# ddemidov/amgcl

Hardware: NVIDIA H100
Metric: cg_iterations_per_second (higher is better)
Workload: dtype f64

## Files before the change

### amgcl_b200/csrc/api_matrices.cu

```cuda
#include "internal.cuh"
#include "csr_kernels.cuh"
#include "csr_launch.cuh"
#include "window.cuh"
#include "offsets.cuh"
#include "patterns.cuh"
#include "narrow.cuh"
#include "values.cuh"

namespace b200 {
int tail_enqueue_csr(b200_ctx_t ctx, int mode, b200_csr_t A, const CsrArgsT<PrecDD> &a);
bool small_csr_accepts(b200_ctx_t ctx, b200_csr_t A);
int small_csr_launch(b200_ctx_t ctx, int mode, b200_csr_t A, const CsrArgsT<PrecDD> &a);
}

using namespace b200;

namespace b200 {

static int choose_lanes(double avg) {
    if (avg <= 12.0) return 1;
    if (avg <= 40.0) return 2;
    if (avg <= 64.0) return 4;
    if (avg <= 160.0) return 8;
    if (avg <= 320.0) return 16;
// ... 427 lines not shown
    A->rows_dist = rd; A->cols_dist = cd;
    A->gather_rows = !rd;
    A->row_off = rows.lo(rank); A->row_B = rows.B;
    A->n_loc = sp.n_loc;
#define DCSR_CUDA(call)                                                        \
    do {                                                                       \
        cudaError_t rc__ = (call);                                             \
        if (rc__ != cudaSuccess) {                                             \
            csr_free(A);                                                       \
            return cuda_fail(rc__, #call, __FILE__, __LINE__);                 \
        }                                                                      \
    } while (0)
    if (cd) {
        A->S = sp.S;
        A->n_send = (int64_t)sp.send_idx.size();
        std::vector<int32_t> idx(sp.send_idx.begin(), sp.send_idx.end());
        DCSR_CUDA(cudaMalloc(&A->send_idx, std::max<size_t>(1, idx.size()) * sizeof(int)));
        const size_t halo_n = std::max<size_t>(2, (size_t)(P * sp.S));
        DCSR_CUDA(cudaMalloc(&A->halo_owned, halo_n * sizeof(double)));
        A->halo = A->halo_owned;
        DCSR_CUDA(cudaMemsetAsync(A->halo, 0, halo_n * sizeof(double), ctx->stream));
        if (!idx.empty())
            DCSR_CUDA(cudaMemcpyAsync(A->send_idx, idx.data(), idx.size() * sizeof(int),
                                      cudaMemcpyHostToDevice, ctx->stream));
        A->bytes += idx.size() * sizeof(int) + (size_t)(P * sp.S) * sizeof(double);
        for (int q = 0; q < P; ++q)
            A->xchg[q] = q != rank && (sp.dep[(size_t)rank * P + q] || sp.dep[(size_t)q * P + rank]);
    }
    if (A->gather_rows && !ctx->p2p) {
        DCSR_CUDA(cudaMalloc((void **)&A->ybuf, ((size_t)P * (size_t)rows.B + 2) * sizeof(double)));
        DCSR_CUDA(cudaMemsetAsync(A->ybuf, 0, ((size_t)P * (size_t)rows.B + 2) * sizeof(double), ctx->stream));
        A->bytes += (size_t)P * (size_t)rows.B * sizeof(double);
    }
    DCSR_CUDA(cudaStreamSynchronize(ctx->stream));
#undef DCSR_CUDA
    if (ctx->p2p) {
        if (cd) {
            size_t half = (size_t)P * (size_t)A->S * sizeof(double);
            half = (std::max<size_t>(half, 16) + 255) & ~size_t(255);
            A->pb_half = half;
            rc = peer_alloc(ctx, kFlagBytes + 2 * half, &A->pb_local, A->pb_peer);
            if (rc) {
                csr_free(A);
                return rc;
            }
            A->bytes += kFlagBytes + 2 * half;
        }
        if (A->gather_rows) {
            size_t half = (size_t)P * (size_t)rows.B * sizeof(double);
            half = (std::max<size_t>(half, 16) + 255) & ~size_t(255);
            A->gb_half = half;
            rc = peer_alloc(ctx, kFlagBytes + 2 * half, &A->gb_local, A->gb_peer);
            if (rc) {
                csr_free(A);
                return rc;
            }
            A->bytes += kFlagBytes + 2 * half;
        }
    }
    *out = A;
    return B200_OK;
}

template <int MODE, int L, bool HALO, class P>
static int launch_csr_LH(b200_ctx_t ctx, b200_csr_t A, const CsrArgsT<P> &args) {
    constexpr bool fp64 = std::is_same<P, PrecDD>::value;
    const StageLayout lay = stage_layout(A->rows_cap, A->nnz_cap, (int)sizeof(typename P::TV));
    if (fp64 && ctx->opt_spmv_variant == 0 && !HALO) {
        const int smem = kHeaderBytes + lay.bytes;
        static bool attr_set[64] = {};
        if (!attr_set[ctx->device & 63]) {
            B200_CUDA(cudaFuncSetAttribute(csr_block_kernel<MODE, L, HALO, PrecDD>,
                                           cudaFuncAttributeMaxDynamicSharedMemorySize, 200 * 1024));
            attr_set[ctx->device & 63] = true;
        }
        csr_block_kernel<MODE, L, HALO, PrecDD><<<(unsigned)A->nblocks, kThreads, smem, ctx->stream>>>(
            *reinterpret_cast<const CsrArgsT<PrecDD> *>(&args));
    } else {
        int rc = B200_OK;
        bool done = false;
        const int fmt = launch_format<P>(ctx, A);
        if constexpr (L <= 4 && !HALO && !IndexedValues<typename P::TV>::value) {
            if (fmt == FMT_PATVAL) {
                rc = launch_ring_pv<MODE, L, P>(ctx, A, args);
                done = true;
            }
        }
        if constexpr (L <= 4) {
            if (fmt == FMT_PATTERN) {
                rc = launch_ring_pat<MODE, L, HALO, P>(ctx, A, args);
                done = true;
            }
        }
        if constexpr (L <= 4) {
            if (fmt == FMT_OFFSET) {
                rc = launch_ring_off<MODE, L, HALO, P>(ctx, A, args);
                done = true;
            }
        }
        if constexpr (L <= 8 && !IndexedValues<typename P::TV>::value) {
            if (fmt == FMT_WINDOW) {
                rc = launch_ring_win<MODE, L, HALO, P>(ctx, A, args);
                done = true;
            }
        }
        if constexpr (L <= 8) {
            if (fmt == FMT_COL16) {
                rc = launch_ring_c16<MODE, L, HALO, P>(ctx, A, args);
                done = true;
            }
            if (fmt == FMT_COL24) {
                rc = launch_ring_c24<MODE, L, HALO, P>(ctx, A, args);
                done = true;
            }
        }
        if (!done) rc = launch_ring_impl<MODE, L, HALO, P, FMT_PLAIN>(ctx, A, args);
        if (rc) return rc;
    }
    B200_CHECK_LAUNCH();
    ctx->launches++;
    return B200_OK;
}

template <int MODE, int L, class P>
static int launch_csr_L(b200_ctx_t ctx, b200_csr_t A, const CsrArgsT<P> &args) {
    if constexpr (!IndexedValues<typename P::TV>::value) {
        if (args.xh) return launch_csr_LH<MODE, L, true, P>(ctx, A, args);
    }
    return launch_csr_LH<MODE, L, false, P>(ctx, A, args);
}

template <int MODE, class P>
static int launch_csr_lanes(b200_ctx_t ctx, b200_csr_t A, const CsrArgsT<P> &args) {
    if (ctx->recording) A->in_graph = true;
    ProfScope prof(ctx, MODE, A->nrows, A->ncols, A->nnz, launch_format<P>(ctx, A), (int)sizeof(typename P::TV));
    switch (A->lanes) {
    case 1:  return launch_csr_L<MODE, 1>(ctx, A, args);
    case 2:  return launch_csr_L<MODE, 2>(ctx, A, args);
    case 4:  return launch_csr_L<MODE, 4>(ctx, A, args);
    case 8:  return launch_csr_L<MODE, 8>(ctx, A, args);
    case 16: return launch_csr_L<MODE, 16>(ctx, A, args);
    default: return launch_csr_L<MODE, 32>(ctx, A, args);
    }
}

template <class PI>
static CsrArgsT<PI> indexed_args(b200_csr_t A, const CsrArgsT<PrecDD> &args) {
    CsrArgsT<PI> s;
    static_assert(sizeof(s) == sizeof(args), "indexed arguments differ from PrecDD only in the value type");
    memcpy(&s, &args, sizeof(s));
    s.val = static_cast<const typename PI::TV *>(A->vidx);
    s.vtab = A->vtab;
    s.vtab_n = A->vtab_n;
    return s;
}

template <int MODE, class P>
static int launch_csr(b200_ctx_t ctx, b200_csr_t A, const CsrArgsT<P> &args) {
    if (A->nblocks == 0) return B200_OK;
    if (std::is_same<P, PrecDD>::value && !args.ndot && !args.xh && !args.gather_on &&
        tail_accepts_csr(ctx, A))
        return tail_enqueue_csr(ctx, MODE, A, *reinterpret_cast<const CsrArgsT<PrecDD> *>(&args));
    {
        const int trc = tail_flush(ctx);
        if (trc) return trc;
    }
    if (std::is_same<P, PrecDD>::value && MODE != MODE_RESID_SCALED && !args.ndot && !args.xh &&
// ... 747 lines not shown
```

### amgcl_b200/csrc/api_patvals.cu

```cuda
#include "csr_launch.cuh"

namespace b200 {

template <int MODE, int L, class P>
int launch_ring_pv(b200_ctx_t ctx, b200_csr_t A, const CsrArgsT<P> &args) {
    return launch_ring_impl<MODE, L, false, P, FMT_PATVAL>(ctx, A, args);
}

#define B200_PV_INST(MODE, P)                                                                        \
    template int launch_ring_pv<MODE, 1, P>(b200_ctx_t, b200_csr_t, const CsrArgsT<P> &);            \
    template int launch_ring_pv<MODE, 2, P>(b200_ctx_t, b200_csr_t, const CsrArgsT<P> &);            \
    template int launch_ring_pv<MODE, 4, P>(b200_ctx_t, b200_csr_t, const CsrArgsT<P> &);

B200_PV_INST(MODE_SPMV, PrecDD)
B200_PV_INST(MODE_SPMV, PrecFF)
B200_PV_INST(MODE_SPMV, PrecFD)
B200_PV_INST(MODE_SPMV, PrecFFD)
B200_PV_INST(MODE_SPMV_ACC, PrecDD)
B200_PV_INST(MODE_SPMV_ACC, PrecFF)
B200_PV_INST(MODE_SPMV_ACC, PrecFD)
B200_PV_INST(MODE_SPMV_ACC, PrecFFD)
B200_PV_INST(MODE_RESID, PrecDD)
B200_PV_INST(MODE_RESID, PrecFF)
B200_PV_INST(MODE_RESID, PrecFD)
B200_PV_INST(MODE_RESID, PrecFDF)
B200_PV_INST(MODE_RESID_SCALED, PrecDD)
B200_PV_INST(MODE_RELAX, PrecDD)
B200_PV_INST(MODE_RELAX, PrecFF)
B200_PV_INST(MODE_RELAX, PrecFD)
B200_PV_INST(MODE_SPMV, PrecSD)
B200_PV_INST(MODE_SPMV_ACC, PrecSD)
B200_PV_INST(MODE_RESID, PrecSD)
B200_PV_INST(MODE_RESID_SCALED, PrecSD)
B200_PV_INST(MODE_RELAX, PrecSD)

}
```

### amgcl_b200/csrc/csr_kernels.cuh

```cuda
#pragma once
#include "common.cuh"
#include "reduce.cuh"
#include <type_traits>

namespace b200 {

enum { FMT_PLAIN = 0,
       FMT_WINDOW = 1,
       FMT_OFFSET = 2,
       FMT_PATTERN = 3,
       FMT_COL16 = 4,
       FMT_COL24 = 5,
       FMT_PATVAL = 6 };
static_assert(FMT_PLAIN == B200_FMT_PLAIN && FMT_WINDOW == B200_FMT_WINDOW && FMT_OFFSET == B200_FMT_OFFSET &&
              FMT_PATTERN == B200_FMT_PATTERN && FMT_COL16 == B200_FMT_COL16 && FMT_COL24 == B200_FMT_COL24 &&
              FMT_PATVAL == B200_FMT_PATVAL,
              "formats as include/amgcl_b200_formats.h reports them");

enum { MODE_SPMV = 0, MODE_SPMV_ACC = 1, MODE_RESID = 2, MODE_RELAX = 3,
       MODE_RESID_SCALED = 4 };

#ifndef B200_GATHER_BATCH
#define B200_GATHER_BATCH 4
#endif
// ... 11 lines not shown
typedef Prec<float, float, float, float, float>      PrecFF;
typedef Prec<float, double, double, double, float>   PrecFD;
typedef Prec<float, double, double, float, float>    PrecFDF;
typedef Prec<float, float, float, double, float>     PrecFFD;
typedef Prec<float, double, double, double, double>  PrecSD;
typedef Prec<unsigned char, double, double, double, double>  PrecI8D;
typedef Prec<unsigned short, double, double, double, double> PrecI16D;

template <class TV> struct IndexedValues : std::false_type {};
template <> struct IndexedValues<unsigned char> : std::true_type {};
template <> struct IndexedValues<unsigned short> : std::true_type {};

template <class TS, class TV>
__device__ __forceinline__ TS value_of(TV v, const double *vtab) {
    if constexpr (IndexedValues<TV>::value) return (TS)vtab[v];
    else return (TS)v;
}

template <class P>
struct CsrArgsT {
    const int    *ptr;
    const unsigned short *ptr16;
    const int    *col;
    const typename P::TV *val;
    const double *vtab;
    int           vtab_n;
    const int4   *blk;
    int           nrows;
    int           nblocks;
    int           rows_cap;
    int           nnz_cap;
    int           row_stream;
    const typename P::TX *x;
    const typename P::TX *xh;
    int           nloc;
    const unsigned long long *wait_flags;
    unsigned int              wait_mask;
    unsigned long long        wait_seq;
    const int                *send_idx;
    int                       n_send;
    int                       nranks;
    typename P::TX           *push_data[kMaxRanks];
    unsigned long long       *push_flag[kMaxRanks];
    unsigned int             *push_ticket;
    unsigned long long        push_seq;
    int                       gather_on;
    typename P::TY           *gather_data[kMaxRanks];
    unsigned long long       *gather_flag[kMaxRanks];
    unsigned int             *gather_ticket;
    unsigned long long        gather_seq;
    const unsigned short *col16;
    const int2   *wrun;
    const int2   *wblk;
    int           run_cap;
    const unsigned char *idx8;
    const int    *off_tab;
    const unsigned char  *pid;
    const unsigned short *pat_start;
    const int    *pat_off;
    int           pat_total;
    const typename P::TV *pat_val;
    const unsigned short *clo16;
    const unsigned char  *chi8;
    const int    *cbase;
    typename P::TY       *y;
    typename P::TX       *xw;
    const typename P::TF *f;
    const typename P::TD *d;
    double        alpha;
    double        beta;
    int           ndot;
    const double *w;
    RedOut        red;
};
typedef CsrArgsT<PrecDD> CsrArgs;

struct StageLayout {
    int val_off, col_off, hi_off, ptr_off, run_off, pid_off, bytes;
};
__host__ __device__ inline StageLayout stage_layout(int rows_cap, int nnz_cap, int val_size,
                                                    int fmt = FMT_PLAIN, int run_cap = 0) {
    StageLayout s;
    s.val_off = 0;
    const bool patval = fmt == FMT_PATVAL;
    int val_bytes = patval ? 0 : nnz_cap * val_size + 16;
    val_bytes = (val_bytes + 15) & ~15;
    s.col_off = s.val_off + val_bytes;
    const bool narrow = fmt == FMT_COL16 || fmt == FMT_COL24;
    int col_bytes = fmt == FMT_WINDOW || narrow ? (nnz_cap + 16) * 2
                  : fmt == FMT_OFFSET  ? (nnz_cap + 32)
                  : fmt == FMT_PATTERN || patval ? 0
                                       : (nnz_cap + 8) * 4;
    col_bytes = (col_bytes + 15) & ~15;
    s.hi_off = s.col_off + col_bytes;
    int hi_bytes = fmt == FMT_COL24 ? nnz_cap + 32 : 0;
    hi_bytes = (hi_bytes + 15) & ~15;
    s.ptr_off = s.hi_off + hi_bytes;
    int ptr_bytes = patval ? 0 : (rows_cap + 16) * 2;
    ptr_bytes = (ptr_bytes + 15) & ~15;
    s.run_off = s.ptr_off + ptr_bytes;
    int run_bytes = fmt == FMT_WINDOW ? (run_cap + 2) * 8 : 0;
    run_bytes = (run_bytes + 15) & ~15;
    s.pid_off = s.run_off + run_bytes;
    int pid_bytes = fmt == FMT_PATTERN || patval ? rows_cap + 32 : 0;
    pid_bytes = (pid_bytes + 15) & ~15;
    s.bytes = s.pid_off + pid_bytes;
    return s;
}
constexpr int kMaxStages   = 8;
constexpr int kHeaderBytes = 448;
constexpr int kWinRunLen   = 64;
constexpr int kOffTabLen   = 256;
constexpr int kPatCap      = 256;
constexpr int kPatOffCap   = 1024;
constexpr int kPatTabBytes = kPatOffCap * 4 + ((kPatCap + 1) * 2 + 15) / 16 * 16;
__host__ __device__ constexpr int fmt_table_bytes(int fmt, int val_size) {
    return fmt == FMT_OFFSET ? kOffTabLen * 4 : fmt == FMT_PATTERN ? kPatTabBytes
         : fmt == FMT_PATVAL ? kPatTabBytes + kPatOffCap * val_size : 0;
}

struct BlockDesc {
    int r0, r1;
    int e0, e1;
    int halo;
    int q0, q1;
    int cb;
};
static_assert(sizeof(BlockDesc) * kMaxStages <= 384 - 128, "descriptors overflow the header");

template <int FMT = FMT_PLAIN, class P>
__device__ __forceinline__ BlockDesc load_desc(const CsrArgsT<P> &a, int b) {
    const int4 q = __ldg(a.blk + b);
    BlockDesc d;
    d.halo = q.x < 0;
    d.r0 = q.x < 0 ? ~q.x : q.x;
    d.r1 = q.y; d.e0 = q.z; d.e1 = q.w;
    d.q0 = d.q1 = 0; d.cb = 0;
    if (FMT == FMT_WINDOW) {
        const int2 w = __ldg(a.wblk + b);
        d.q0 = w.x; d.q1 = w.y;
    }
    if (FMT == FMT_COL16 || FMT == FMT_COL24) d.cb = __ldg(a.cbase + b);
    return d;
}

template <int FMT = FMT_PLAIN, class P>
__device__ __forceinline__ bool issue_block(const CsrArgsT<P> &a, const BlockDesc &d, char *stage,
                                            const StageLayout &lay, uint64_t *bar,
                                            uint64_t policy) {
    typedef typename P::TV TV;
    constexpr int VA = 16 / (int)sizeof(TV);
    const int nnz = d.e1 - d.e0;
    if (FMT == FMT_PLAIN && nnz > a.nnz_cap) {
        asm volatile("mbarrier.arrive.shared::cta.b64 _, [%0];" ::"r"(ptx::smem_addr(bar))
                     : "memory");
        return false;
    }
    constexpr bool PV = FMT == FMT_PATVAL;
    const int a0 = d.e0 & ~(VA - 1);
    const int nval = PV ? 0 : ((d.e1 - a0) + VA - 1) & ~(VA - 1);
    const int p0 = d.r0 & ~7;
    const int nptr = PV ? 0 : ((d.r1 + 1 - p0) + 7) & ~7;
    int ncol = 0, nhi = 0, nrun = 0, npid = 0;
    const void *csrc = nullptr, *hsrc = nullptr, *psrc = nullptr;
    if (FMT == FMT_PLAIN) {
        const int c0 = d.e0 & ~3;
        ncol = (((d.e1 - c0) + 3) & ~3) * 4;
        csrc = a.col + c0;
    } else if (FMT == FMT_WINDOW || FMT == FMT_COL16 || FMT == FMT_COL24) {
        const int c0 = d.e0 & ~7;
        ncol = (((d.e1 - c0) + 7) & ~7) * 2;
        csrc = (FMT == FMT_WINDOW ? a.col16 : a.clo16) + c0;
    } else if (FMT == FMT_OFFSET) {
        const int c0 = d.e0 & ~15;
        ncol = ((d.e1 - c0) + 15) & ~15;
        csrc = a.idx8 + c0;
    }
    if (FMT == FMT_COL24) {
        const int h0 = d.e0 & ~15;
        nhi = ((d.e1 - h0) + 15) & ~15;
        hsrc = a.chi8 + h0;
    }
    if (FMT == FMT_WINDOW) {
        const int qa = d.q0 & ~1;
        nrun = (((d.q1 - qa) + 1) & ~1) * 8;
        psrc = a.wrun + qa;
    }
    if (FMT == FMT_PATTERN || PV) {
        const int q0 = d.r0 & ~15;
        npid = ((d.r1 - q0) + 15) & ~15;
        psrc = a.pid + q0;
    }
    const uint32_t bytes = nval * (int)sizeof(TV) + ncol + nhi + nptr * 2 + nrun + npid;
    ptx::mbar_expect_tx(bar, bytes);
    if (nval) ptx::bulk_g2s(stage + lay.val_off, a.val + a0, nval * (int)sizeof(TV), bar, policy);
    if (ncol) ptx::bulk_g2s(stage + lay.col_off, csrc, ncol, bar, policy);
    if (nhi) ptx::bulk_g2s(stage + lay.hi_off, hsrc, nhi, bar, policy);
    if (nptr) ptx::bulk_g2s(stage + lay.ptr_off, a.ptr16 + p0, nptr * 2, bar, policy);
    if (nrun) ptx::bulk_g2s(stage + lay.run_off, psrc, nrun, bar, policy);
    if (npid) ptx::bulk_g2s(stage + lay.pid_off, psrc, npid, bar, policy);
    return true;
}

struct RowAcc { double s0, s1; };

template <class P>
struct RowOps {
    typename P::TF f;
    typename P::TD d;
    typename P::TX x;
    typename P::TY y;
    double         w;
};
template <int MODE, class P>
__device__ __forceinline__ RowOps<P> load_row_ops(const CsrArgsT<P> &a, int r) {
    RowOps<P> o;
    o.f = 0; o.d = 0; o.x = 0; o.y = 0; o.w = 0.0;
    if (MODE == MODE_SPMV_ACC) o.y = a.y[r];
    if (MODE == MODE_RESID || MODE == MODE_RESID_SCALED || MODE == MODE_RELAX) o.f = a.f[r];
    if (MODE == MODE_RESID_SCALED || MODE == MODE_RELAX) o.d = a.d[r];
    if (MODE == MODE_RELAX) o.x = a.x[r];
    if (a.ndot && a.w) o.w = a.w[r];
    return o;
}

template <int MODE, class P>
__device__ __forceinline__ void store_row(const CsrArgsT<P> &a, int r, typename P::TY sum, RowAcc &acc,
                                          const RowOps<P> &o) {
    typedef typename P::TY TY;
    TY out;
    double wv = 0.0;
    if (MODE == MODE_SPMV) {
        out = (TY)(a.alpha * sum);
    } else if (MODE == MODE_SPMV_ACC) {
        out = (TY)(a.alpha * sum + a.beta * o.y);
    } else if (MODE == MODE_RESID) {
        out = (TY)(o.f - sum);
    } else if (MODE == MODE_RESID_SCALED) {
        const typename P::TF fr = o.f;
        out = (TY)(fr - sum);
        a.xw[r] = fma((typename P::TX)(a.alpha * o.d), (typename P::TX)fr, (typename P::TX)0);
    } else {
        const typename P::TF fr = o.f;
        const TY t = (TY)(fr - sum);
        const TY w = (TY)(a.alpha * o.d);
        out = fma(w, t, (TY)o.x);
        wv = (double)fr;
    }
    a.y[r] = out;
    if (a.gather_on) {
#pragma unroll 1
        for (int q = 0; q < a.nranks; ++q)
            if (a.gather_data[q]) a.gather_data[q][r] = out;
    }
    if (a.ndot) {
        const double yv = (double)out;
        if (a.w) wv = o.w;
        else if (MODE != MODE_RELAX) wv = yv;
        acc.s0 = fma(yv, wv, acc.s0);
        if (a.ndot > 1) acc.s1 = fma(yv, yv, acc.s1);
    }
}
template <int MODE, class P>
__device__ __forceinline__ void store_row(const CsrArgsT<P> &a, int r, typename P::TY sum, RowAcc &acc) {
    store_row<MODE>(a, r, sum, acc, load_row_ops<MODE>(a, r));
}

template <bool HALO, class P>
__device__ __forceinline__ typename P::TX gather(const CsrArgsT<P> &a,
                                                 const typename P::TX *__restrict__ x, int c) {
    if (HALO) {
        if (c < a.nloc) return __ldg(x + c);
        return __ldcg(a.xh + (c - a.nloc));
    }
    return __ldg(x + c);
}

template <int MODE, bool HALO, class P>
__device__ __forceinline__ typename P::TX gather_m(const CsrArgsT<P> &a,
                                                   const typename P::TX *__restrict__ x, int c) {
    typedef typename P::TX TX;
    if (MODE == MODE_RESID_SCALED)
        return fma((TX)(a.alpha * __ldg(a.d + c)), (TX)__ldg(a.f + c), (TX)0);
    return gather<HALO>(a, x, c);
}

template <bool HALO, class P>
__device__ __forceinline__ void wait_for_halo(const CsrArgsT<P> &a, const BlockDesc &d) {
    if (!HALO) return;
    if (!d.halo || !a.wait_mask) return;
    if (threadIdx.x == 0) {
        unsigned int m = a.wait_mask;
        while (m) {
            const int q = __ffs(m) - 1;
            m &= m - 1;
            unsigned long long v;
            do {
                asm volatile("ld.acquire.sys.global.u64 %0, [%1];" : "=l"(v) : "l"(a.wait_flags + q) : "memory");
            } while (v < a.wait_seq);
        }
    }
    __syncthreads();
}

template <int MODE, bool HALO, class P>
__device__ __forceinline__ void fill_window(const CsrArgsT<P> &a, const BlockDesc &d, const char *stage,
                                            const StageLayout &lay, typename P::TX *win) {
    const int2 *runs = reinterpret_cast<const int2 *>(stage + lay.run_off) + (d.q0 & 1);
    const int nq   = d.q1 - d.q0;
    const int lane = threadIdx.x & 31;
    const typename P::TX *__restrict__ x = a.x;
    for (int q = threadIdx.x >> 5; q < nq; q += kThreads / 32) {
        const int2 rn   = runs[q];
        const int first = rn.x;
        const int len   = rn.y & 0xffff;
        const int slot  = (int)((unsigned)rn.y >> 16);
#pragma unroll
        for (int i = lane; i < kWinRunLen; i += 32)
            if (i < len) win[slot + i] = gather_m<MODE, HALO>(a, x, first + i);
    }
    __syncthreads();
}

template <int MODE, int L, bool HALO, class P, int FMT = FMT_PLAIN>
__device__ __forceinline__ void compute_staged(const CsrArgsT<P> &a, const BlockDesc &d,
                                               const char *stage, const StageLayout &lay, RowAcc &acc,
                                               const typename P::TX *win = nullptr, const int *off = nullptr,
                                               const unsigned short *pstart = nullptr, int k0 = 0,
                                               const double *vtab = nullptr,
                                               const typename P::TV *pval = nullptr) {
    constexpr bool WIN = FMT == FMT_WINDOW;
    constexpr bool OFF = FMT == FMT_OFFSET;
    constexpr bool PV  = FMT == FMT_PATVAL;
    constexpr bool PAT = FMT == FMT_PATTERN || PV;
    constexpr bool NAR = FMT == FMT_COL16 || FMT == FMT_COL24;
    typedef typename P::TV TV;
    typedef typename P::TX TX;
    typedef typename P::TY TS;
    typedef typename std::conditional<WIN || NAR, unsigned short,
                                      typename std::conditional<OFF, unsigned char, int>::type>::type CI;
    static_assert(!((WIN || OFF || PAT || NAR) && L >= 16), "compressed column formats use at most 8 lanes per row");
    const unsigned char *pid_s = reinterpret_cast<const unsigned char *>(stage + lay.pid_off) + (d.r0 & 15);
    constexpr int VA = 16 / (int)sizeof(TV);
    const TV *val_s = reinterpret_cast<const TV *>(stage + lay.val_off);
    const CI     *col_s = reinterpret_cast<const CI *>(stage + lay.col_off);
    const unsigned char  *hi_s  = reinterpret_cast<const unsigned char *>(stage + lay.hi_off);
    const unsigned short *ptr_s = reinterpret_cast<const unsigned short *>(stage + lay.ptr_off) + (d.r0 & 7);
    const int vo = d.e0 & ~(VA - 1);
    const int nr = d.r1 - d.r0;
    const int co = WIN || NAR ? (d.e0 & ~7) : OFF ? (d.e0 & ~15) : (d.e0 & ~3);
    const int ho = d.e0 & ~15;
    auto stored_col = [&](int e) -> int {
        if (!NAR) return col_s[e - co];
        if (FMT == FMT_COL24) return d.cb + ((int)col_s[e - co] | (int)hi_s[e - ho] << 16);
        return d.cb + (int)col_s[e - co];
    };
    auto row_beg = [&](int rr) -> int { return d.e0 + (int)ptr_s[rr]; };
    auto row_end = [&](int rr) -> int { return d.e0 + (int)ptr_s[rr + 1] + (rr + 1 == nr ? d.e1 - d.e0 : 0); };
    constexpr int G = kThreads / L;
    const int c0   = (((int)threadIdx.x >> 5) - k0) & (kThreads / 32 - 1);
    const int g    = (threadIdx.x & 31) / L;
    const int lane = threadIdx.x % L;
    const TX *__restrict__ x = a.x;

    if (L >= 16) {
        constexpr int RU = kGatherBatch;
        for (int base = c0 * (32 / L); base < nr; base += G * RU) {
            int  beg[RU], end[RU], c[RU];
            TV   v[RU];
            TX   xv[RU];
            TS   sum[RU];
            bool rowok[RU], p[RU];
#pragma unroll
            for (int u = 0; u < RU; ++u) {
                const int rr = base + u * G + g;
                rowok[u] = rr < nr;
                beg[u] = rowok[u] ? row_beg(rr) : 0;
                end[u] = rowok[u] ? row_end(rr) : 0;
                sum[u] = 0;
            }
#pragma unroll
            for (int u = 0; u < RU; ++u) {
                const int e = beg[u] + lane;
                p[u] = e < end[u];
                c[u] = p[u] ? stored_col(e) : 0;
                v[u] = p[u] ? val_s[e - vo] : (TV)0;
            }
#pragma unroll
            for (int u = 0; u < RU; ++u) xv[u] = p[u] ? gather_m<MODE, HALO>(a, x, c[u]) : (TX)0;
#pragma unroll
            for (int u = 0; u < RU; ++u)
                if (p[u]) sum[u] = value_of<TS>(v[u], vtab) * (TS)xv[u];
#pragma unroll
            for (int u = 0; u < RU; ++u)
                for (int e = beg[u] + lane + L; e < end[u]; e += L)
                    sum[u] = fma(value_of<TS>(val_s[e - vo], vtab), (TS)gather_m<MODE, HALO>(a, x, stored_col(e)),
                                 sum[u]);
#pragma unroll
            for (int o = L / 2; o > 0; o >>= 1) {
#pragma unroll
                for (int u = 0; u < RU; ++u) sum[u] += __shfl_xor_sync(0xffffffffu, sum[u], o);
            }
#pragma unroll
            for (int u = 0; u < RU; ++u)
                if (rowok[u] && lane == 0) store_row<MODE>(a, d.r0 + base + u * G + g, sum[u], acc);
        }
    } else
    for (int base = c0 * (32 / L); base < nr; base += G) {
        const int  rr    = base + g;
        const bool valid = rr < nr;
        TS sum = 0;
        RowOps<P> ops;
        ops.f = 0; ops.d = 0; ops.x = 0; ops.y = 0; ops.w = 0.0;
        if (valid) {
            if (lane == 0) ops = load_row_ops<MODE>(a, d.r0 + rr);
            const int beg = PV ? (int)pstart[pid_s[rr]] : row_beg(rr);
            const int end = PV ? (int)pstart[pid_s[rr] + 1] : row_end(rr);
            int pb = 0;
            if (PAT && !PV) pb = (int)pstart[pid_s[rr]] - beg;
            constexpr int U = (L == 1) ? 2 * kGatherBatch : kGatherBatch;
            for (int e = beg + lane; e < end; e += U * L) {
                int  c[U];
                TX   xv[U];
                bool p[U];
#pragma unroll
                for (int u = 0; u < U; ++u) {
                    const int eu = e + u * L;
                    p[u] = eu < end;
                    if (PAT) c[u] = d.r0 + rr + off[pb + (p[u] ? eu : e)];
                    else c[u] = stored_col(p[u] ? eu : e);
                }
                if (OFF) {
#pragma unroll
                    for (int u = 0; u < U; ++u) c[u] = d.r0 + rr + off[c[u]];
                }
#pragma unroll
                for (int u = 0; u < U; ++u)
                    xv[u] = !p[u] ? (TX)0 : WIN ? win[c[u]] : gather_m<MODE, HALO>(a, x, c[u]);
#pragma unroll
                for (int u = 0; u < U; ++u)
                    if (p[u]) sum = fma(value_of<TS>(PV ? pval[e + u * L] : val_s[e + u * L - vo], vtab), (TS)xv[u], sum);
            }
        }
        if (L > 1) {
#pragma unroll
            for (int o = L / 2; o > 0; o >>= 1) sum += __shfl_xor_sync(0xffffffffu, sum, o);
        }
        if (valid && lane == 0) store_row<MODE>(a, d.r0 + rr, sum, acc, ops);
    }
}

template <int MODE, bool HALO, class P>
__device__ __forceinline__ void compute_long(const CsrArgsT<P> &a, const BlockDesc &d,
                                             double *red_s , RowAcc &acc) {
    typedef typename P::TX TX;
    typedef typename P::TY TS;
    const TX *__restrict__ x = a.x;
    for (int r = d.r0; r < d.r1; ++r) {
        const int beg = __ldg(a.ptr + r), end = __ldg(a.ptr + r + 1);
        TS sum = 0;
        for (int e = beg + threadIdx.x; e < end; e += kThreads)
            sum = fma(value_of<TS>(__ldg(a.val + e), a.vtab), (TS)gather_m<MODE, HALO>(a, x, __ldg(a.col + e)), sum);
#pragma unroll
        for (int o = 16; o > 0; o >>= 1) sum += __shfl_xor_sync(0xffffffffu, sum, o);
        __syncthreads();
        if ((threadIdx.x & 31) == 0) red_s[threadIdx.x >> 5] = (double)sum;
        __syncthreads();
        if (threadIdx.x == 0) {
            TS tot = 0;
#pragma unroll
            for (int w = 0; w < kThreads / 32; ++w) tot += (TS)red_s[w];
            store_row<MODE>(a, r, tot, acc);
        }
    }
}

__device__ __forceinline__ void xchg_st_release_sys(unsigned long long *p, unsigned long long v) {
    asm volatile("st.release.sys.global.u64 [%0], %1;" ::"l"(p), "l"(v) : "memory");
}
template <class P>
__device__ __forceinline__ void halo_push(const CsrArgsT<P> &a) {
    if (!a.push_seq) return;
    const typename P::TX *__restrict__ x = a.x;
    for (int i = blockIdx.x * kThreads + threadIdx.x; i < a.n_send; i += gridDim.x * kThreads) {
        const typename P::TX v = x[a.send_idx[i]];
#pragma unroll 1
        for (int q = 0; q < a.nranks; ++q)
            if (a.push_data[q]) a.push_data[q][i] = v;
    }
    __threadfence_system();
    __shared__ bool push_last;
    __syncthreads();
    if (threadIdx.x == 0) {
        const unsigned int done = atomicAdd(a.push_ticket, 1u);
        push_last = (done == gridDim.x - 1);
    }
    __syncthreads();
    if (push_last) {
        if (threadIdx.x < a.nranks && a.push_flag[threadIdx.x])
            xchg_st_release_sys(a.push_flag[threadIdx.x], a.push_seq);
        if (threadIdx.x == 0) *a.push_ticket = 0;
    }
}
template <class P>
__device__ __forceinline__ void gather_finish(const CsrArgsT<P> &a) {
    __threadfence_system();
    __shared__ bool gather_last;
    __syncthreads();
    if (threadIdx.x == 0) {
        const unsigned int done = atomicAdd(a.gather_ticket, 1u);
        gather_last = (done == gridDim.x - 1);
    }
    __syncthreads();
    if (gather_last) {
        if (threadIdx.x < a.nranks && a.gather_flag[threadIdx.x])
            xchg_st_release_sys(a.gather_flag[threadIdx.x], a.gather_seq);
        if (threadIdx.x == 0) *a.gather_ticket = 0;
    }
}

template <int MODE, int L, bool HALO, class P>
__global__ void __launch_bounds__(kThreads, 4) csr_block_kernel(const CsrArgsT<P> a) {
    extern __shared__ __align__(128) char smem[];
    uint64_t *bar   = reinterpret_cast<uint64_t *>(smem);
    double   *red_s = reinterpret_cast<double *>(smem + 64);
    char     *stage = smem + kHeaderBytes;
    const StageLayout lay = stage_layout(a.rows_cap, a.nnz_cap, (int)sizeof(typename P::TV));

    const int b = blockIdx.x;
    const BlockDesc d = load_desc(a, b);
    const bool staged = (d.e1 - d.e0) <= a.nnz_cap;
    RowAcc acc = {0.0, 0.0};

    if (staged) {
        if (threadIdx.x == 0) {
            ptx::mbar_init(bar, 1);
            ptx::fence_mbar_init();
            issue_block(a, d, stage, lay, bar, ptx::policy_evict_first());
        }
        __syncthreads();
        ptx::mbar_wait(bar, 0);
        wait_for_halo<HALO>(a, d);
        compute_staged<MODE, L, HALO>(a, d, stage, lay, acc);
    } else {
        wait_for_halo<HALO>(a, d);
        compute_long<MODE, HALO>(a, d, red_s, acc);
    }
}

template <int MODE, int L, bool HALO, class P, int FMT = FMT_PLAIN>
__global__ void __launch_bounds__(kThreads, 4) csr_ring_kernel(const CsrArgsT<P> a, const int nstages) {
    extern __shared__ __align__(128) char smem[];
    uint64_t  *bars  = reinterpret_cast<uint64_t *>(smem);
    double    *red_s = reinterpret_cast<double *>(smem + 64);
    BlockDesc *descs = reinterpret_cast<BlockDesc *>(smem + 128);
    unsigned  *done  = reinterpret_cast<unsigned *>(smem + 384);
    const StageLayout lay = stage_layout(a.rows_cap, a.nnz_cap, (int)sizeof(typename P::TV), FMT, a.run_cap);
    char *stages = smem + kHeaderBytes;
    typename P::TX *win = reinterpret_cast<typename P::TX *>(stages + (size_t)nstages * lay.bytes);
    int *off_s = reinterpret_cast<int *>(stages + (size_t)nstages * lay.bytes);
    unsigned short *pstart_s = reinterpret_cast<unsigned short *>(off_s + kPatOffCap);
    typename P::TV *pval_s = reinterpret_cast<typename P::TV *>(stages + (size_t)nstages * lay.bytes + kPatTabBytes);
    constexpr bool IDX = IndexedValues<typename P::TV>::value;
    static_assert(!(IDX && (HALO || FMT == FMT_WINDOW || FMT == FMT_PATVAL)),
                  "indexed values: single-GPU, fixed-size tables only, values streamed");
    static_assert(!(HALO && FMT == FMT_PATVAL), "value-keyed patterns: single-GPU only");
    double *vtab_s = reinterpret_cast<double *>(stages + (size_t)nstages * lay.bytes +
                                                fmt_table_bytes(FMT, (int)sizeof(typename P::TV)));

    const int first = blockIdx.x;
    const int step  = gridDim.x;
    const int mine  = (a.nblocks - first + step - 1) / step;
    const uint64_t policy = ptx::policy_evict_first();

    if (threadIdx.x == 0) {
        for (int s = 0; s < nstages; ++s) { ptx::mbar_init(bars + s, 1); done[s] = 0; }
        ptx::fence_mbar_init();
        const int pre = mine < nstages ? mine : nstages;
        for (int i = 0; i < pre; ++i) {
            const BlockDesc d = load_desc<FMT>(a, first + i * step);
            descs[i] = d;
            issue_block<FMT>(a, d, stages + (size_t)i * lay.bytes, lay, bars + i, policy);
        }
    }
    if constexpr (FMT == FMT_OFFSET) {
        static_assert(kOffTabLen == kThreads, "one table entry per thread");
        off_s[threadIdx.x] = __ldg(a.off_tab + threadIdx.x);
    }
    if constexpr (FMT == FMT_PATTERN || FMT == FMT_PATVAL) {
        for (int i = threadIdx.x; i < a.pat_total; i += kThreads) off_s[i] = __ldg(a.pat_off + i);
        for (int i = threadIdx.x; i <= kPatCap; i += kThreads) pstart_s[i] = __ldg(a.pat_start + i);
    }
    if constexpr (FMT == FMT_PATVAL) {
        for (int i = threadIdx.x; i < a.pat_total; i += kThreads) pval_s[i] = __ldg(a.pat_val + i);
    }
    if constexpr (IDX) {
        for (int i = threadIdx.x; i < a.vtab_n; i += kThreads) vtab_s[i] = __ldg(a.vtab + i);
    }
    __syncthreads();
    ptx::pdl_wait();
    if (HALO) halo_push(a);

    const bool decoupled = FMT == FMT_OFFSET || FMT == FMT_PATTERN || FMT == FMT_PATVAL ||
                           (FMT != FMT_WINDOW && a.row_stream);
    constexpr int LS = FMT == FMT_PLAIN || L < 16 ? L : 8;
    RowAcc acc = {0.0, 0.0};
    int k0 = 0;
    int s = 0, parity = 0;
    for (int i = 0; i < mine; ++i) {
        ptx::mbar_wait(bars + s, parity);
        const BlockDesc d = descs[s];
        wait_for_halo<HALO>(a, d);
        const char *stage = stages + (size_t)s * lay.bytes;
        if constexpr (FMT == FMT_WINDOW) {
            fill_window<MODE, HALO>(a, d, stage, lay, win);
            compute_staged<MODE, LS, HALO, P, FMT_WINDOW>(a, d, stage, lay, acc, win);
        } else if (FMT != FMT_PLAIN || (d.e1 - d.e0) <= a.nnz_cap) {
            compute_staged<MODE, LS, HALO, P, FMT>(a, d, stage, lay, acc, nullptr, off_s, pstart_s, k0, vtab_s, pval_s);
            k0 += (d.r1 - d.r0 + 32 / LS - 1) / (32 / LS);
        } else {
            compute_long<MODE, HALO>(a, d, red_s, acc);
        }
        if (decoupled) {
            __syncwarp();
            if ((threadIdx.x & 31) == 0) {
                __threadfence_block();
                const unsigned arrived = atomicAdd(done + s, 1u);
                if (arrived == kThreads / 32 - 1) {
                    done[s] = 0;
                    __threadfence_block();
                    if (i + nstages < mine) {
                        const BlockDesc n = load_desc<FMT>(a, first + (i + nstages) * step);
                        descs[s] = n;
                        issue_block<FMT>(a, n, stages + (size_t)s * lay.bytes, lay, bars + s, policy);
                    }
                }
            }
        } else {
            __syncthreads();
            if (threadIdx.x == 0 && i + nstages < mine) {
                const BlockDesc n = load_desc<FMT>(a, first + (i + nstages) * step);
                descs[s] = n;
                issue_block<FMT>(a, n, stages + (size_t)s * lay.bytes, lay, bars + s, policy);
            }
        }
        if (++s == nstages) { s = 0; parity ^= 1; }
    }
    if (HALO && a.gather_on) gather_finish(a);
    if (a.ndot) {
        double v[2] = {acc.s0, acc.s1};
        red_finish<2>(a.red, v);
    }
}

template <class TD, class TF, class TX>
__global__ void __launch_bounds__(kThreads) relax_zero_kernel(size_t n, double omega,
                                                              const TD *__restrict__ d,
                                                              const TF *__restrict__ f,
                                                              TX *__restrict__ x) {
    ptx::pdl_wait();
    const size_t stride = (size_t)gridDim.x * blockDim.x;
    for (size_t i = (size_t)blockIdx.x * blockDim.x + threadIdx.x; i < n; i += stride) {
        x[i] = fma((TX)(omega * d[i]), (TX)f[i], (TX)0);
    }
}

}
```

### amgcl_b200/csrc/csr_launch.cuh

```cuda
#pragma once
#include "internal.cuh"
#include "csr_kernels.cuh"

namespace b200 {

inline int ring_budget(int ctas) { return 228 * 1024 / ctas - 1024 - 1536; }

inline int value_table_bytes(int count) { return (count * (int)sizeof(double) + 15) & ~15; }

inline bool value_index_fits(b200_ctx_t ctx, int rows_cap, int nnz_cap, int fmt, int idx_bytes, int count) {
    const StageLayout lay = stage_layout(rows_cap, nnz_cap, idx_bytes, fmt);
    return fmt != FMT_WINDOW && ctx->opt_stages >= 1 &&
           kHeaderBytes + (int)ctx->opt_stages * lay.bytes + fmt_table_bytes(fmt, idx_bytes) + value_table_bytes(count) <=
               ring_budget((int)ctx->opt_ctas_per_sm);
}

template <class P>
inline int ring_smem(b200_ctx_t ctx, b200_csr_t A, int fmt, int *stages_out) {
    const StageLayout lay = stage_layout(A->rows_cap, A->nnz_cap, (int)sizeof(typename P::TV), fmt, A->win_runs);
    const int extra = (fmt == FMT_WINDOW ? (int)(((size_t)A->win_slots * sizeof(typename P::TX) + 15) & ~(size_t)15)
                                         : fmt_table_bytes(fmt, (int)sizeof(typename P::TV))) +
                      (IndexedValues<typename P::TV>::value ? value_table_bytes(A->vtab_n) : 0);
    int stages = (int)ctx->opt_stages;
    const int per_cta_budget = ring_budget((int)ctx->opt_ctas_per_sm);
    while (stages > 1 && kHeaderBytes + stages * lay.bytes + extra > per_cta_budget) --stages;
    *stages_out = stages;
    const int smem = kHeaderBytes + stages * lay.bytes + extra;
    return (fmt == FMT_WINDOW && smem > per_cta_budget) ? 0 : smem;
}

template <int MODE, int L, bool HALO, class P, int FMT>
inline int launch_ring_impl(b200_ctx_t ctx, b200_csr_t A, const CsrArgsT<P> &args) {
    int stages = 1;
    const int smem = ring_smem<P>(ctx, A, FMT, &stages);
    static bool attr_set[64] = {};
    if (!attr_set[ctx->device & 63]) {
        cudaFuncAttributes fa;
        B200_CUDA(cudaFuncGetAttributes(&fa, csr_ring_kernel<MODE, L, HALO, P, FMT>));
        B200_CUDA(cudaFuncSetAttribute(csr_ring_kernel<MODE, L, HALO, P, FMT>,
                                       cudaFuncAttributeMaxDynamicSharedMemorySize,
                                       227 * 1024 - (int)fa.sharedSizeBytes));
        attr_set[ctx->device & 63] = true;
    }
    const int64_t cap = (int64_t)ctx->sm_count * ctx->opt_ctas_per_sm;
    const unsigned grid = (unsigned)std::min<int64_t>(A->nblocks, cap);
    B200_CUDA(launch_pdl(ctx, csr_ring_kernel<MODE, L, HALO, P, FMT>, dim3(grid), dim3(kThreads), (size_t)smem,
                         args, stages));
    return B200_OK;
}

template <int MODE, int L, bool HALO, class P>
int launch_ring_win(b200_ctx_t ctx, b200_csr_t A, const CsrArgsT<P> &args);
template <int MODE, int L, bool HALO, class P>
int launch_ring_off(b200_ctx_t ctx, b200_csr_t A, const CsrArgsT<P> &args);
template <int MODE, int L, bool HALO, class P>
int launch_ring_pat(b200_ctx_t ctx, b200_csr_t A, const CsrArgsT<P> &args);
template <int MODE, int L, class P>
int launch_ring_pv(b200_ctx_t ctx, b200_csr_t A, const CsrArgsT<P> &args);
template <int MODE, int L, bool HALO, class P>
int launch_ring_c16(b200_ctx_t ctx, b200_csr_t A, const CsrArgsT<P> &args);
template <int MODE, int L, bool HALO, class P>
int launch_ring_c24(b200_ctx_t ctx, b200_csr_t A, const CsrArgsT<P> &args);

inline int stored_format(b200_csr_t A) {
    if (A->pid) return A->pat_val ? FMT_PATVAL : FMT_PATTERN;
    if (A->idx8) return FMT_OFFSET;
    if (A->col16) return FMT_WINDOW;
    if (A->narrow) return A->narrow == 24 ? FMT_COL24 : FMT_COL16;
    return FMT_PLAIN;
}

template <class TV>
inline const TV *pattern_values(b200_csr_t A) {
    if constexpr (std::is_same<TV, double>::value) return A->pat_val;
    else if constexpr (std::is_same<TV, float>::value) return A->pat_val32;
    else return nullptr;
}

template <class P>
inline int launch_format(b200_ctx_t ctx, b200_csr_t A) {
    if (ctx->opt_spmv_variant != 1) return FMT_PLAIN;
    if (A->pid && ctx->opt_patterns && A->lanes <= 4) {
        const int vs = (int)sizeof(typename P::TV);
        if (pattern_values<typename P::TV>(A) && ctx->opt_pattern_values && ctx->opt_stages >= 1 &&
            kHeaderBytes + (int)ctx->opt_stages * stage_layout(A->rows_cap, A->nnz_cap, vs, FMT_PATVAL).bytes +
                    fmt_table_bytes(FMT_PATVAL, vs) <= ring_budget((int)ctx->opt_ctas_per_sm))
            return FMT_PATVAL;
        return FMT_PATTERN;
    }
    if (A->idx8 && ctx->opt_offsets && A->lanes <= 4) return FMT_OFFSET;
    if (A->col16 && ctx->opt_window && A->lanes <= 8 && A->win_runs >= 1) {
        int stages;
        if (ring_smem<P>(ctx, A, FMT_WINDOW, &stages) != 0) return FMT_WINDOW;
    }
    if (A->narrow && ctx->opt_narrow && A->lanes <= 8) return A->narrow == 24 ? FMT_COL24 : FMT_COL16;
    return FMT_PLAIN;
}

}
```

Measured before the change: 457.3.

## Run value-keyed pattern SpMV in a dedicated ring-free kernel with batched rows

Value-keyed pattern matrices no longer go through the staged ring kernel. They now use a dedicated csr_patval_kernel. It keeps only the pattern offset and value tables in shared memory, walks rows directly without staging, and processes two rows per thread group at once. It also prefetches the next rows' pattern ids through an evict-first, no-L1-allocate load. The intent is to remove the staging overhead and raise memory-level parallelism in the gathers. The cost is a separate code path and more registers per thread, with the kernel targeting four CTAs per SM.

```diff
diff --git a/amgcl_b200/csrc/api_matrices.cu b/amgcl_b200/csrc/api_matrices.cu
--- a/amgcl_b200/csrc/api_matrices.cu
+++ b/amgcl_b200/csrc/api_matrices.cu
@@ -533,7 +533,7 @@
         const int fmt = launch_format<P>(ctx, A);
         if constexpr (L <= 4 && !HALO && !IndexedValues<typename P::TV>::value) {
             if (fmt == FMT_PATVAL) {
-                rc = launch_ring_pv<MODE, L, P>(ctx, A, args);
+                rc = launch_patval<MODE, L, P>(ctx, A, args);
                 done = true;
             }
         }
diff --git a/amgcl_b200/csrc/api_patvals.cu b/amgcl_b200/csrc/api_patvals.cu
--- a/amgcl_b200/csrc/api_patvals.cu
+++ b/amgcl_b200/csrc/api_patvals.cu
@@ -3,14 +3,18 @@
 namespace b200 {
 
 template <int MODE, int L, class P>
-int launch_ring_pv(b200_ctx_t ctx, b200_csr_t A, const CsrArgsT<P> &args) {
-    return launch_ring_impl<MODE, L, false, P, FMT_PATVAL>(ctx, A, args);
+int launch_patval(b200_ctx_t ctx, b200_csr_t A, const CsrArgsT<P> &args) {
+    const int smem = fmt_table_bytes(FMT_PATVAL, (int)sizeof(typename P::TV));
+    const int64_t cap = (int64_t)ctx->sm_count * ctx->opt_ctas_per_sm;
+    const unsigned grid = (unsigned)std::min<int64_t>(A->nblocks, cap);
+    B200_CUDA(launch_pdl(ctx, csr_patval_kernel<MODE, L, P>, dim3(grid), dim3(kThreads), (size_t)smem, args));
+    return B200_OK;
 }
 
 #define B200_PV_INST(MODE, P)                                                                        \
-    template int launch_ring_pv<MODE, 1, P>(b200_ctx_t, b200_csr_t, const CsrArgsT<P> &);            \
-    template int launch_ring_pv<MODE, 2, P>(b200_ctx_t, b200_csr_t, const CsrArgsT<P> &);            \
-    template int launch_ring_pv<MODE, 4, P>(b200_ctx_t, b200_csr_t, const CsrArgsT<P> &);
+    template int launch_patval<MODE, 1, P>(b200_ctx_t, b200_csr_t, const CsrArgsT<P> &);             \
+    template int launch_patval<MODE, 2, P>(b200_ctx_t, b200_csr_t, const CsrArgsT<P> &);             \
+    template int launch_patval<MODE, 4, P>(b200_ctx_t, b200_csr_t, const CsrArgsT<P> &);
 
 B200_PV_INST(MODE_SPMV, PrecDD)
 B200_PV_INST(MODE_SPMV, PrecFF)
diff --git a/amgcl_b200/csrc/csr_kernels.cuh b/amgcl_b200/csrc/csr_kernels.cuh
--- a/amgcl_b200/csrc/csr_kernels.cuh
+++ b/amgcl_b200/csrc/csr_kernels.cuh
@@ -117,27 +117,26 @@
                                                     int fmt = FMT_PLAIN, int run_cap = 0) {
     StageLayout s;
     s.val_off = 0;
-    const bool patval = fmt == FMT_PATVAL;
-    int val_bytes = patval ? 0 : nnz_cap * val_size + 16;
+    int val_bytes = nnz_cap * val_size + 16;
     val_bytes = (val_bytes + 15) & ~15;
     s.col_off = s.val_off + val_bytes;
     const bool narrow = fmt == FMT_COL16 || fmt == FMT_COL24;
     int col_bytes = fmt == FMT_WINDOW || narrow ? (nnz_cap + 16) * 2
                   : fmt == FMT_OFFSET  ? (nnz_cap + 32)
-                  : fmt == FMT_PATTERN || patval ? 0
+                  : fmt == FMT_PATTERN ? 0
                                        : (nnz_cap + 8) * 4;
     col_bytes = (col_bytes + 15) & ~15;
     s.hi_off = s.col_off + col_bytes;
     int hi_bytes = fmt == FMT_COL24 ? nnz_cap + 32 : 0;
     hi_bytes = (hi_bytes + 15) & ~15;
     s.ptr_off = s.hi_off + hi_bytes;
-    int ptr_bytes = patval ? 0 : (rows_cap + 16) * 2;
+    int ptr_bytes = (rows_cap + 16) * 2;
     ptr_bytes = (ptr_bytes + 15) & ~15;
     s.run_off = s.ptr_off + ptr_bytes;
     int run_bytes = fmt == FMT_WINDOW ? (run_cap + 2) * 8 : 0;
     run_bytes = (run_bytes + 15) & ~15;
     s.pid_off = s.run_off + run_bytes;
-    int pid_bytes = fmt == FMT_PATTERN || patval ? rows_cap + 32 : 0;
+    int pid_bytes = fmt == FMT_PATTERN ? rows_cap + 32 : 0;
     pid_bytes = (pid_bytes + 15) & ~15;
     s.bytes = s.pid_off + pid_bytes;
     return s;
@@ -191,11 +190,10 @@
                      : "memory");
         return false;
     }
-    constexpr bool PV = FMT == FMT_PATVAL;
     const int a0 = d.e0 & ~(VA - 1);
-    const int nval = PV ? 0 : ((d.e1 - a0) + VA - 1) & ~(VA - 1);
+    const int nval = ((d.e1 - a0) + VA - 1) & ~(VA - 1);
     const int p0 = d.r0 & ~7;
-    const int nptr = PV ? 0 : ((d.r1 + 1 - p0) + 7) & ~7;
+    const int nptr = ((d.r1 + 1 - p0) + 7) & ~7;
     int ncol = 0, nhi = 0, nrun = 0, npid = 0;
     const void *csrc = nullptr, *hsrc = nullptr, *psrc = nullptr;
     if (FMT == FMT_PLAIN) {
@@ -221,7 +219,7 @@
         nrun = (((d.q1 - qa) + 1) & ~1) * 8;
         psrc = a.wrun + qa;
     }
-    if (FMT == FMT_PATTERN || PV) {
+    if (FMT == FMT_PATTERN) {
         const int q0 = d.r0 & ~15;
         npid = ((d.r1 - q0) + 15) & ~15;
         psrc = a.pid + q0;
@@ -362,12 +360,10 @@
                                                const char *stage, const StageLayout &lay, RowAcc &acc,
                                                const typename P::TX *win = nullptr, const int *off = nullptr,
                                                const unsigned short *pstart = nullptr, int k0 = 0,
-                                               const double *vtab = nullptr,
-                                               const typename P::TV *pval = nullptr) {
+                                               const double *vtab = nullptr) {
     constexpr bool WIN = FMT == FMT_WINDOW;
     constexpr bool OFF = FMT == FMT_OFFSET;
-    constexpr bool PV  = FMT == FMT_PATVAL;
-    constexpr bool PAT = FMT == FMT_PATTERN || PV;
+    constexpr bool PAT = FMT == FMT_PATTERN;
     constexpr bool NAR = FMT == FMT_COL16 || FMT == FMT_COL24;
     typedef typename P::TV TV;
     typedef typename P::TX TX;
@@ -449,10 +445,10 @@
         ops.f = 0; ops.d = 0; ops.x = 0; ops.y = 0; ops.w = 0.0;
         if (valid) {
             if (lane == 0) ops = load_row_ops<MODE>(a, d.r0 + rr);
-            const int beg = PV ? (int)pstart[pid_s[rr]] : row_beg(rr);
-            const int end = PV ? (int)pstart[pid_s[rr] + 1] : row_end(rr);
+            const int beg = row_beg(rr);
+            const int end = row_end(rr);
             int pb = 0;
-            if (PAT && !PV) pb = (int)pstart[pid_s[rr]] - beg;
+            if (PAT) pb = (int)pstart[pid_s[rr]] - beg;
             constexpr int U = (L == 1) ? 2 * kGatherBatch : kGatherBatch;
             for (int e = beg + lane; e < end; e += U * L) {
                 int  c[U];
@@ -474,7 +470,7 @@
                     xv[u] = !p[u] ? (TX)0 : WIN ? win[c[u]] : gather_m<MODE, HALO>(a, x, c[u]);
 #pragma unroll
                 for (int u = 0; u < U; ++u)
-                    if (p[u]) sum = fma(value_of<TS>(PV ? pval[e + u * L] : val_s[e + u * L - vo], vtab), (TS)xv[u], sum);
+                    if (p[u]) sum = fma(value_of<TS>(val_s[e + u * L - vo], vtab), (TS)xv[u], sum);
             }
         }
         if (L > 1) {
@@ -595,11 +591,9 @@
     typename P::TX *win = reinterpret_cast<typename P::TX *>(stages + (size_t)nstages * lay.bytes);
     int *off_s = reinterpret_cast<int *>(stages + (size_t)nstages * lay.bytes);
     unsigned short *pstart_s = reinterpret_cast<unsigned short *>(off_s + kPatOffCap);
-    typename P::TV *pval_s = reinterpret_cast<typename P::TV *>(stages + (size_t)nstages * lay.bytes + kPatTabBytes);
     constexpr bool IDX = IndexedValues<typename P::TV>::value;
-    static_assert(!(IDX && (HALO || FMT == FMT_WINDOW || FMT == FMT_PATVAL)),
-                  "indexed values: single-GPU, fixed-size tables only, values streamed");
-    static_assert(!(HALO && FMT == FMT_PATVAL), "value-keyed patterns: single-GPU only");
+    static_assert(FMT != FMT_PATVAL, "value-keyed patterns run csr_patval_kernel");
+    static_assert(!(IDX && (HALO || FMT == FMT_WINDOW)), "indexed values: single-GPU, fixed-size tables only");
     double *vtab_s = reinterpret_cast<double *>(stages + (size_t)nstages * lay.bytes +
                                                 fmt_table_bytes(FMT, (int)sizeof(typename P::TV)));
 
@@ -622,12 +616,9 @@
         static_assert(kOffTabLen == kThreads, "one table entry per thread");
         off_s[threadIdx.x] = __ldg(a.off_tab + threadIdx.x);
     }
-    if constexpr (FMT == FMT_PATTERN || FMT == FMT_PATVAL) {
+    if constexpr (FMT == FMT_PATTERN) {
         for (int i = threadIdx.x; i < a.pat_total; i += kThreads) off_s[i] = __ldg(a.pat_off + i);
         for (int i = threadIdx.x; i <= kPatCap; i += kThreads) pstart_s[i] = __ldg(a.pat_start + i);
-    }
-    if constexpr (FMT == FMT_PATVAL) {
-        for (int i = threadIdx.x; i < a.pat_total; i += kThreads) pval_s[i] = __ldg(a.pat_val + i);
     }
     if constexpr (IDX) {
         for (int i = threadIdx.x; i < a.vtab_n; i += kThreads) vtab_s[i] = __ldg(a.vtab + i);
@@ -636,7 +627,7 @@
     ptx::pdl_wait();
     if (HALO) halo_push(a);
 
-    const bool decoupled = FMT == FMT_OFFSET || FMT == FMT_PATTERN || FMT == FMT_PATVAL ||
+    const bool decoupled = FMT == FMT_OFFSET || FMT == FMT_PATTERN ||
                            (FMT != FMT_WINDOW && a.row_stream);
     constexpr int LS = FMT == FMT_PLAIN || L < 16 ? L : 8;
     RowAcc acc = {0.0, 0.0};
@@ -651,7 +642,7 @@
             fill_window<MODE, HALO>(a, d, stage, lay, win);
             compute_staged<MODE, LS, HALO, P, FMT_WINDOW>(a, d, stage, lay, acc, win);
         } else if (FMT != FMT_PLAIN || (d.e1 - d.e0) <= a.nnz_cap) {
-            compute_staged<MODE, LS, HALO, P, FMT>(a, d, stage, lay, acc, nullptr, off_s, pstart_s, k0, vtab_s, pval_s);
+            compute_staged<MODE, LS, HALO, P, FMT>(a, d, stage, lay, acc, nullptr, off_s, pstart_s, k0, vtab_s);
             k0 += (d.r1 - d.r0 + 32 / LS - 1) / (32 / LS);
         } else {
             compute_long<MODE, HALO>(a, d, red_s, acc);
@@ -688,6 +679,130 @@
     }
 }
 
+
+template <int MODE> struct PatvalBatch { static constexpr int R = MODE == MODE_RESID_SCALED ? 1 : 2; };
+
+__device__ __forceinline__ int ld_pid(const unsigned char *p, uint64_t policy) {
+    unsigned v;
+    asm volatile("ld.global.nc.L1::no_allocate.L2::cache_hint.u8 %0, [%1], %2;" : "=r"(v) : "l"(p), "l"(policy));
+    return (int)v;
+}
+
+template <int MODE, int L, class P>
+__global__ void __launch_bounds__(kThreads, 4) csr_patval_kernel(const CsrArgsT<P> a) {
+    typedef typename P::TV TV;
+    typedef typename P::TX TX;
+    typedef typename P::TY TS;
+    static_assert(L == 1 || L == 2 || L == 4, "value-keyed patterns: 1, 2 or 4 lanes per row");
+    static_assert(!IndexedValues<TV>::value, "value-keyed patterns keep the values themselves");
+    constexpr int R  = PatvalBatch<MODE>::R;
+    constexpr int K  = L == 1 ? 2 * kGatherBatch : kGatherBatch;
+    constexpr int CR = 32 / L;
+    constexpr int NW = kThreads / 32;
+    extern __shared__ __align__(128) char smem[];
+    int *off_s = reinterpret_cast<int *>(smem);
+    unsigned short *pstart_s = reinterpret_cast<unsigned short *>(off_s + kPatOffCap);
+    TV *pval_s = reinterpret_cast<TV *>(smem + kPatTabBytes);
+
+    const int first = blockIdx.x;
+    const int step  = gridDim.x;
+    const int mine  = (a.nblocks - first + step - 1) / step;
+    const int warp  = threadIdx.x >> 5;
+    const int wl    = threadIdx.x & 31;
+    const int g     = wl / L;
+    const int lane  = threadIdx.x % L;
+
+    auto block_rows = [&](int i) -> int2 {
+        if (i >= mine) return make_int2(0, 0);
+        const int4 q = __ldg(a.blk + first + i * step);
+        return make_int2(q.x, q.y);
+    };
+    int2 win_n = block_rows(wl), win_c = make_int2(0, 0);
+    int i = -1, r0 = 0, r1 = 0, k0 = 0, j = 0;
+    auto next_row = [&]() -> int {
+        while (j * CR >= r1 - r0) {
+            k0 += (r1 - r0 + CR - 1) / CR;
+            if (++i >= mine) return -2;
+            if ((i & 31) == 0) { win_c = win_n; win_n = block_rows(i + 32 + wl); }
+            r0 = __shfl_sync(0xffffffffu, win_c.x, i & 31);
+            r1 = __shfl_sync(0xffffffffu, win_c.y, i & 31);
+            j = (warp - k0) & (NW - 1);
+        }
+        const int r = r0 + j * CR + g;
+        j += NW;
+        return r < r1 ? r : -1;
+    };
+
+    const uint64_t policy = ptx::policy_evict_first();
+    for (int e = threadIdx.x; e < a.pat_total; e += kThreads) {
+        off_s[e] = __ldg(a.pat_off + e);
+        pval_s[e] = __ldg(a.pat_val + e);
+    }
+    for (int e = threadIdx.x; e <= kPatCap; e += kThreads) pstart_s[e] = __ldg(a.pat_start + e);
+    int row[R], pid[R];
+#pragma unroll
+    for (int u = 0; u < R; ++u) row[u] = next_row();
+#pragma unroll
+    for (int u = 0; u < R; ++u) pid[u] = row[u] >= 0 ? ld_pid(a.pid + row[u], policy) : 0;
+    __syncthreads();
+    ptx::pdl_wait();
+
+    const TX *__restrict__ x = a.x;
+    RowAcc acc = {0.0, 0.0};
+    while (row[0] != -2) {
+        int nrow[R], npid[R];
+#pragma unroll
+        for (int u = 0; u < R; ++u) nrow[u] = next_row();
+#pragma unroll
+        for (int u = 0; u < R; ++u) npid[u] = nrow[u] >= 0 ? ld_pid(a.pid + nrow[u], policy) : 0;
+        RowOps<P> ops[R];
+        int beg[R], end[R], len = 0;
+        TS sum[R];
+#pragma unroll
+        for (int u = 0; u < R; ++u) {
+            const bool valid = row[u] >= 0;
+            ops[u] = valid && lane == 0 ? load_row_ops<MODE>(a, row[u]) : RowOps<P>{};
+            beg[u] = valid ? (int)pstart_s[pid[u]] : 0;
+            end[u] = valid ? (int)pstart_s[pid[u] + 1] : 0;
+            len = max(len, end[u] - beg[u]);
+            sum[u] = 0;
+        }
+        for (int k = lane; k < len; k += K * L) {
+            TX xv[R][K];
+#pragma unroll
+            for (int u = 0; u < R; ++u)
+#pragma unroll
+                for (int q = 0; q < K; ++q) {
+                    const int e = beg[u] + k + q * L;
+                    xv[u][q] = e < end[u] ? gather_m<MODE, false>(a, x, row[u] + off_s[e]) : (TX)0;
+                }
+#pragma unroll
+            for (int u = 0; u < R; ++u)
+#pragma unroll
+                for (int q = 0; q < K; ++q) {
+                    const int e = beg[u] + k + q * L;
+                    if (e < end[u]) sum[u] = fma((TS)pval_s[e], (TS)xv[u][q], sum[u]);
+                }
+        }
+        if (L > 1) {
+#pragma unroll
+            for (int o = L / 2; o > 0; o >>= 1) {
+#pragma unroll
+                for (int u = 0; u < R; ++u) sum[u] += __shfl_xor_sync(0xffffffffu, sum[u], o);
+            }
+        }
+#pragma unroll
+        for (int u = 0; u < R; ++u)
+            if (row[u] >= 0 && lane == 0) store_row<MODE>(a, row[u], sum[u], acc, ops[u]);
+#pragma unroll
+        for (int u = 0; u < R; ++u) { row[u] = nrow[u]; pid[u] = npid[u]; }
+    }
+    if (a.ndot) {
+        double v[2] = {acc.s0, acc.s1};
+        red_finish<2>(a.red, v);
+    }
+}
+
 template <class TD, class TF, class TX>
 __global__ void __launch_bounds__(kThreads) relax_zero_kernel(size_t n, double omega,
                                                               const TD *__restrict__ d,
diff --git a/amgcl_b200/csrc/csr_launch.cuh b/amgcl_b200/csrc/csr_launch.cuh
--- a/amgcl_b200/csrc/csr_launch.cuh
+++ b/amgcl_b200/csrc/csr_launch.cuh
@@ -56,7 +56,7 @@
 template <int MODE, int L, bool HALO, class P>
 int launch_ring_pat(b200_ctx_t ctx, b200_csr_t A, const CsrArgsT<P> &args);
 template <int MODE, int L, class P>
-int launch_ring_pv(b200_ctx_t ctx, b200_csr_t A, const CsrArgsT<P> &args);
+int launch_patval(b200_ctx_t ctx, b200_csr_t A, const CsrArgsT<P> &args);
 template <int MODE, int L, bool HALO, class P>
 int launch_ring_c16(b200_ctx_t ctx, b200_csr_t A, const CsrArgsT<P> &args);
 template <int MODE, int L, bool HALO, class P>
@@ -80,14 +80,8 @@
 template <class P>
 inline int launch_format(b200_ctx_t ctx, b200_csr_t A) {
     if (ctx->opt_spmv_variant != 1) return FMT_PLAIN;
-    if (A->pid && ctx->opt_patterns && A->lanes <= 4) {
-        const int vs = (int)sizeof(typename P::TV);
-        if (pattern_values<typename P::TV>(A) && ctx->opt_pattern_values && ctx->opt_stages >= 1 &&
-            kHeaderBytes + (int)ctx->opt_stages * stage_layout(A->rows_cap, A->nnz_cap, vs, FMT_PATVAL).bytes +
-                    fmt_table_bytes(FMT_PATVAL, vs) <= ring_budget((int)ctx->opt_ctas_per_sm))
-            return FMT_PATVAL;
-        return FMT_PATTERN;
-    }
+    if (A->pid && ctx->opt_patterns && A->lanes <= 4)
+        return pattern_values<typename P::TV>(A) && ctx->opt_pattern_values ? FMT_PATVAL : FMT_PATTERN;
     if (A->idx8 && ctx->opt_offsets && A->lanes <= 4) return FMT_OFFSET;
     if (A->col16 && ctx->opt_window && A->lanes <= 8 && A->win_runs >= 1) {
         int stages;
```

Result: faster. 480.7 (median of 6 runs) (+5.1%).
